# snphbaum/scikit-gpuppy

Hardware: AMD Instinct MI355X
Metric: GP fit+predict pts/sec (K+Cholesky, N=16384 d=8) (higher is better)
Workload: dtype f64; 1 GPU; C3: N=16384 d=8 M=16384 fit(Gram+Cholesky+alpha)+estimate_many, theta fixed; global_batch=32768, parallelism=1 GPU

## Files before the change

scikit-gpuppy_amd/csrc/chol.hip:

```cpp
#include <algorithm>
#include <atomic>
#include <chrono>
#include <cstdio>
#include <cstdlib>
#include <functional>
#include <map>
#include <mutex>
#include <vector>

#include "common.h"

#include "leaf.h"

__attribute__((amdgpu_waves_per_eu(2, 2))) __global__ __launch_bounds__(256) void potrf_trtri128_elim_kernel(double *A, long ld, double *dinv, double *diag_out, int *info,
                                                                 int col_offset, int prio)
{
    __shared__ __attribute__((aligned(16))) double X[36 * XB];
    __shared__ int bad_s;
    if (prio) __builtin_amdgcn_s_setprio(3);
    leaf_elim_body(A, ld, dinv, diag_out, info, col_offset, X, &bad_s);
}

static void leaf_exclusive_setup()
{
    static const bool done = [] {
        (void)hipFuncSetAttribute(reinterpret_cast<const void *>(potrf_trtri128_elim_kernel), hipFuncAttributeMaxDynamicSharedMemorySize, 52 * 1024);
        return true;
    }();
    (void)done;
}

int launch_potrf_leaf(double *A, int64_t ld, double *dinv, double *diag_out, int *info_dev, int col_offset,
                      hipStream_t s, Profiler *prof, int exclusive)
{
    ProfScope ps(prof, s, GPX_K_POTRF_LEAF, (double)TILE * TILE * TILE);
    if (exclusive) leaf_exclusive_setup();
    hipLaunchKernelGGL(potrf_trtri128_elim_kernel, dim3(1), dim3(256), exclusive ? 52 * 1024 : 0, s, A, (long)ld, dinv, diag_out, info_dev, col_offset, 1);
    GPX_HIP(hipGetLastError());
    return 0;
}

extern "C" int gpx_dev_potrf_leaf(double *A, int64_t ld, double *dinv, double *diag_out, int *info_dev, int col_offset,
                                  void *stream)
{
    return launch_potrf_leaf(A, ld, dinv, diag_out, info_dev, col_offset, (hipStream_t)stream, nullptr, 0);
}

static inline int64_t split_point(int64_t nb)
{
    int64_t h = 1;
    while (h * 2 < nb) h *= 2;
    return h;
}

int trsm_right_lt(double *Z, int64_t ldz, int64_t rows, const double *L, int64_t ldl, const double *Dinv,
                  int64_t c0, int64_t c1, hipStream_t s, Profiler *prof)
{
    const int64_t nb = c1 - c0;
    if (nb <= 0 || rows <= 0) return 0;
    if (nb == 1) {
        double *Zc = Z + c0 * TILE;
        return launch_gemm_nt(Zc, ldz, Dinv + c0 * (int64_t)TILE * TILE, TILE, Zc, ldz, rows, TILE, TILE, 1.0, 0.0, 0, s, prof);
    }
    const int64_t h = split_point(nb), cm = c0 + h;
    GPX_TRY(trsm_right_lt(Z, ldz, rows, L, ldl, Dinv, c0, cm, s, prof));
    GPX_TRY(launch_gemm_nt(Z + c0 * TILE, ldz, L + (cm * TILE) * ldl + c0 * TILE, ldl, Z + cm * TILE, ldz, rows,
                           (c1 - cm) * TILE, h * TILE, -1.0, 1.0, 0, s, prof));
    return trsm_right_lt(Z, ldz, rows, L, ldl, Dinv, cm, c1, s, prof);
}

static int trtri_upper_rec(double *Z, int64_t ldz, const double *L, int64_t ldl, const double *Dinv, int64_t c0, int64_t c1,
                           hipStream_t s, Profiler *prof)
{
    const int64_t nb = c1 - c0;
    if (nb <= 0) return 0;
    if (nb == 1) {
        double *Zc = Z + c0 * TILE;
        return launch_gemm_nt(Zc, ldz, Dinv + c0 * (int64_t)TILE * TILE, TILE, Zc, ldz, c1 * TILE, TILE, TILE, 1.0, 0.0, 0, s, prof);
    }
    const int64_t h = split_point(nb), cm = c0 + h;
    GPX_TRY(trtri_upper_rec(Z, ldz, L, ldl, Dinv, c0, cm, s, prof));
    GPX_TRY(launch_gemm_nt(Z + c0 * TILE, ldz, L + (cm * TILE) * ldl + c0 * TILE, ldl, Z + cm * TILE, ldz, cm * TILE,
                           (c1 - cm) * TILE, h * TILE, -1.0, 1.0, 0, s, prof, (int)(c0 * TILE) + 1));
    return trtri_upper_rec(Z, ldz, L, ldl, Dinv, cm, c1, s, prof);
}

int build_linv_t(const double *L, int64_t ld, int64_t nblk, const double *Dinv, double *Z, hipStream_t s, Profiler *prof)
{
    const int64_t npad = nblk * TILE;
    GPX_TRY(launch_set_identity(Z, npad, npad, s));
    return trtri_upper_rec(Z, npad, L, ld, Dinv, 0, nblk, s, prof);
}

int build_kinv_from_factor(const double *L, int64_t ld, int64_t nblk, const double *Dinv, double *Z, double *Kinv,
                           hipStream_t s, Profiler *prof)
{
    const int64_t npad = nblk * TILE;
    GPX_TRY(build_linv_t(L, ld, nblk, Dinv, Z, s, prof));
    GPX_TRY(launch_gemm_nt(Z, npad, Z, npad, Kinv, npad, npad, npad, npad, 1.0, 0.0, 1, s, prof, 1));
    return launch_symmetrize_lower(Kinv, npad, npad, s);
}

static int chol_rec(double *L, int64_t ld, int64_t b0, int64_t b1, double *Dinv, double *diagL, int *info_dev,
                    hipStream_t s, Profiler *prof)
{
    const int64_t nb = b1 - b0;
    if (nb <= 0) return 0;
    if (nb == 1)
        return launch_potrf_leaf(L + (b0 * TILE) * ld + b0 * TILE, ld, Dinv + b0 * (int64_t)TILE * TILE,
                                 diagL + b0 * TILE, info_dev, (int)(b0 * TILE), s, prof, 0);
    const int64_t h = split_point(nb), bm = b0 + h;
    GPX_TRY(chol_rec(L, ld, b0, bm, Dinv, diagL, info_dev, s, prof));
    GPX_TRY(trsm_right_lt(L + (bm * TILE) * ld, ld, (b1 - bm) * TILE, L, ld, Dinv, b0, bm, s, prof));
    const double *A21 = L + (bm * TILE) * ld + b0 * TILE;
    GPX_TRY(launch_gemm_nt(A21, ld, A21, ld, L + (bm * TILE) * ld + bm * TILE, ld, (b1 - bm) * TILE, (b1 - bm) * TILE,
                           h * TILE, -1.0, 1.0, 1, s, prof));
    return chol_rec(L, ld, bm, b1, Dinv, diagL, info_dev, s, prof);
}

constexpr int64_t CHOL_NBP = 8;

int64_t chol_dataflow_state_ints(int64_t nbr);
int64_t chol_dataflow_table_ints(int64_t nbr);
bool chol_dataflow_supported(int64_t nbr);
int64_t chol_dataflow_word_steps();
int64_t chol_dataflow_word_colc(int64_t nbr, int64_t k);
int launch_chol_dataflow(double *L, int64_t ld, int64_t nb, int64_t c0, double *Dinv, double *diag, int *info_dev, int *state_dev,
                         std::vector<int> &host_tab, unsigned long long limit_ticks, hipStream_t s, int workers = 0, int exclusive = 0,
                         const int *tab_ready = nullptr, int first_rows = 0, int extra = 0, const int *gate = nullptr);
int chol_dataflow_fill_tables(int nbr, int first_rows, int *dst, int cap);

static_assert(CHOL_NBP * TILE == CHOL_PANEL_COLS, "common.h: CHOL_PANEL_COLS");

static long env_long(const char *name, long dflt) { const char *e = getenv(name); return e ? atol(e) : dflt; }
static bool debug_enabled() { static const bool v = getenv("GPX_DEBUG") != nullptr; return v; }

static unsigned long long wait_limit_ticks()
{
    static const unsigned long long v = [] { const char *e = getenv("GPX_WAIT_LIMIT_MS"); const double ms = e ? atof(e) : 5000.0; return (unsigned long long)((ms > 0.01 ? ms : 0.01) * 1e5); }();
    return v;
}

__global__ void wait_count_kernel(const int *ctr, int want, unsigned long long limit_ticks, int *stall)
{
    const unsigned long long t0 = __builtin_amdgcn_s_memrealtime();
    while (__hip_atomic_load(ctr, __ATOMIC_RELAXED, __HIP_MEMORY_SCOPE_AGENT) < want) {
        if (__builtin_amdgcn_s_memrealtime() - t0 > limit_ticks) {
            __hip_atomic_store(stall, 1, __ATOMIC_RELAXED, __HIP_MEMORY_SCOPE_AGENT);
            break;
        }
        __builtin_amdgcn_s_sleep(8);
    }
}

static int queue_wait(hipStream_t on, const int *counter, int want, int *stall, unsigned long long limit_ticks = wait_limit_ticks())
{
    hipLaunchKernelGGL(wait_count_kernel, dim3(1), dim3(1), 0, on, counter, want, limit_ticks, stall);
    GPX_HIP(hipGetLastError());
    return 0;
}

struct Events {
    std::vector<hipEvent_t> all;
    Events() = default;
    Events(const Events &) = delete;
    Events &operator=(const Events &) = delete;
    ~Events() { clear(); }
    void clear()
    {
        for (hipEvent_t e : all) (void)hipEventDestroy(e);
        all.clear();
    }
    int make(hipEvent_t *e)
    {
        GPX_HIP(hipEventCreateWithFlags(e, hipEventDisableTiming));
        all.push_back(*e);
        return 0;
    }
};

struct TopPipe {
    hipStream_t stream = nullptr;
    int64_t r0 = 0, r1 = 0;
    Events *events = nullptr;
    const int *colsig = nullptr;
    int colwant = 0;
    int *stall = nullptr;
    const int *sq_state = nullptr;
    int64_t sq_rows = 0;
    int64_t sq_nbr = 0;
    const TopPipe *next = nullptr;
    void follow_square(const int *state, int64_t rows, int64_t below)
    {
        sq_state = state;
        sq_rows = rows;
        sq_nbr = rows + below;
    }
};

static int colsig_wait(const TopPipe *top, int64_t c)
{
    static const bool force_stall = getenv("GPX_TEST_FORCE_STALL") != nullptr;
    static bool forced = false;
    const bool force = force_stall && !forced;
    forced = forced || force;
    return queue_wait(top->stream, top->colsig + c, force ? 0x7fffffff : top->colwant, top->stall, force ? 1000ull : wait_limit_ticks());
}

static int top_column(double *L, int64_t ld, int64_t B0, int64_t j, const double *Dinv, const TopPipe *top, Profiler *prof, int part = 0)
{
    double *Zt = L + (top->r0 * TILE) * ld;
    const int64_t M = (top->r1 - top->r0) * TILE;
    if (top->sq_state && part == 1) return 0;
    if (top->colsig && part != 2) {
        if (!top->sq_state) GPX_TRY(colsig_wait(top, j - B0));
        else if (j == B0)
            for (int64_t c = 0; c < top->sq_rows; ++c) GPX_TRY(colsig_wait(top, c));
    }
    if (top->sq_state) {
        const int64_t B1 = B0 + top->sq_rows;
        GPX_TRY(queue_wait(top->stream, top->sq_state + chol_dataflow_word_steps(), (int)(j - B0 + 1), top->stall));
        GPX_TRY(launch_gemm_nt(Zt + j * TILE, ld, Dinv + j * (int64_t)TILE * TILE, TILE, Zt + j * TILE, ld, M, TILE, TILE, 1.0, 0.0, 0, top->stream, prof));
        if (j + 1 < B1) {
            GPX_TRY(queue_wait(top->stream, top->sq_state + chol_dataflow_word_colc(top->sq_nbr, j - B0), (int)(4 * (B1 - 1 - j)), top->stall));
            GPX_TRY(launch_gemm_nt(Zt + j * TILE, ld, L + ((j + 1) * TILE) * ld + j * TILE, ld, Zt + (j + 1) * TILE, ld, M, (B1 - 1 - j) * TILE, TILE,
                                   -1.0, 1.0, 0, top->stream, prof, 0, 0, 1));
        }
        return 0;
    }
    if (j > B0 && part != 2)
        GPX_TRY(launch_gemm_nt(Zt + B0 * TILE, ld, L + (j * TILE) * ld + B0 * TILE, ld, Zt + j * TILE, ld, M, TILE, (j - B0) * TILE,
                               -1.0, 1.0, 0, top->stream, prof));
    if (part == 1) return 0;
    return launch_gemm_nt(Zt + j * TILE, ld, Dinv + j * (int64_t)TILE * TILE, TILE, Zt + j * TILE, ld, M, TILE, TILE, 1.0, 0.0, 0,
                          top->stream, prof);
}

static int chol_square_steps(double *L, int64_t ld, int64_t B0, int64_t B1, int64_t j0, int64_t j1, double *Dinv,
                             double *diagL, int *info_dev, hipStream_t s, Profiler *prof, const TopPipe *top = nullptr, int excl = 0)
{
    for (int64_t j = j0; j < j1; ++j) {
        for (const TopPipe *t = top; t; t = t->next)
            if (t->stream && t->r1 > t->r0) GPX_TRY(top_column(L, ld, B0, j, Dinv, t, prof, 1));
        GPX_TRY(launch_potrf_leaf(L + (j * TILE) * ld + j * TILE, ld, Dinv + j * (int64_t)TILE * TILE, diagL + j * TILE, info_dev,
                                  (int)(j * TILE), s, prof, excl == 2 || (excl == 1 && j == B0)));
        const int64_t rows_below = B1 - (j + 1);
        if (rows_below > 0) {
            double *Z = L + ((j + 1) * TILE) * ld + j * TILE;
            GPX_TRY(launch_gemm_nt(Z, ld, Dinv + j * (int64_t)TILE * TILE, TILE, Z, ld, rows_below * TILE, TILE, TILE, 1.0, 0.0, 0, s, prof));
            GPX_TRY(launch_gemm_nt(Z, ld, Z, ld, L + ((j + 1) * TILE) * ld + (j + 1) * TILE, ld, rows_below * TILE,
                                   rows_below * TILE, TILE, -1.0, 1.0, 0, s, prof));
        }
        hipEvent_t e = nullptr;
        for (const TopPipe *t = top; t; t = t->next) {
            if (!t->stream || t->r1 <= t->r0) continue;
            if (!e) {
                GPX_TRY(t->events->make(&e));
                GPX_HIP(hipEventRecord(e, s));
            }
            GPX_HIP(hipStreamWaitEvent(t->stream, e, 0));
            GPX_TRY(top_column(L, ld, B0, j, Dinv, t, prof, 2));
        }
    }
    return 0;
}

int chol_panel_factor(double *L, int64_t ld, int64_t nblk_all, int64_t B0, int64_t B1, double *Dinv, double *diagL,
                      int *info_dev, hipStream_t s, Profiler *prof)
{
    GPX_TRY(chol_square_steps(L, ld, B0, B1, B0, B1, Dinv, diagL, info_dev, s, prof));
    if (nblk_all > B1)
        GPX_TRY(trsm_right_lt(L + (B1 * TILE) * ld, ld, (nblk_all - B1) * TILE, L, ld, Dinv, B0, B1, s, prof));
    return 0;
}

static void retire_events(const std::vector<hipEvent_t> &fresh)
{
    static std::mutex mu;
    static std::vector<hipEvent_t> pending;
    std::lock_guard<std::mutex> lk(mu);
    size_t keep = 0;
    for (size_t i = 0; i < pending.size(); ++i) {
        if (hipEventQuery(pending[i]) == hipSuccess) (void)hipEventDestroy(pending[i]);
        else pending[keep++] = pending[i];
    }
    pending.resize(keep);
    pending.insert(pending.end(), fresh.begin(), fresh.end());
}

static void retire_buffers(const std::vector<void *> &bufs, const std::vector<hipStream_t> &behind)
{
    static std::mutex mu;
    struct Pending { std::vector<hipEvent_t> events; std::vector<void *> bufs; };
    static std::vector<Pending> pending;
    std::lock_guard<std::mutex> lk(mu);
    size_t keep = 0;
    for (size_t i = 0; i < pending.size(); ++i) {
        bool done = true;
        for (hipEvent_t e : pending[i].events) done = done && hipEventQuery(e) == hipSuccess;
        if (done) {
            for (hipEvent_t e : pending[i].events) (void)hipEventDestroy(e);
            for (void *q : pending[i].bufs) dfree(q);
        } else {
            if (keep != i) pending[keep] = std::move(pending[i]);
            ++keep;
        }
    }
    pending.resize(keep);
    if (bufs.empty()) return;
    Pending fresh;
    fresh.bufs = bufs;
    for (hipStream_t st : behind) {
        hipEvent_t e = nullptr;
        if (hipEventCreateWithFlags(&e, hipEventDisableTiming) != hipSuccess || hipEventRecord(e, st) != hipSuccess) {
            (void)hipStreamSynchronize(st);
            if (e) (void)hipEventDestroy(e);
            continue;
        }
        fresh.events.push_back(e);
    }
    pending.push_back(std::move(fresh));
}

__global__ void merge_info_kernel(const int *two, int *one)
{
    if (two[1]) atomicMax(one, (int)GPX_INFO_STALLED);
    else if (two[0]) atomicCAS(one, 0, two[0]);
}

static thread_local int g_panel_share = 1;
extern "C" int gpx_dev_set_panel_share(int ranks)
{
    if (ranks < 1) { gpx_set_error("gpx_dev_set_panel_share: ranks must be >= 1"); return GPX_ERR_BAD_ARG; }
    g_panel_share = ranks;
    return 0;
}

static long sqk_from() { static const long v = env_long("GPX_SQK_FROM", -2); return v; }
static bool square_launch_wanted(int64_t b0, int64_t beside, int share, bool from_p)
{
    static const long tiles = env_long("GPX_SQK_TILES", 1000);
    if (sqk_from() == -1 || !chol_dataflow_supported(CHOL_NBP)) return false;
    if (sqk_from() == 0) return true;
    if (sqk_from() > 0 && from_p) return b0 >= sqk_from() * CHOL_NBP;
    return b0 == 0 || beside / share < tiles;
}

int chol_panel_factor_piped(double *L, int64_t ld, int64_t nblk_all, int64_t B0, int64_t B1, double *Dinv, double *diagL,
                            int *info_dev, hipStream_t s, Profiler *prof, const double *P, int64_t ldp, int64_t kp,
                            int64_t hb, hipStream_t sh, hipStream_t sf)
{
    const int64_t c0 = B0 * TILE, w = (B1 - B0) * TILE;
    const bool own_streams = sh && sf;
    double *Csq = L + c0 * ld + c0;
    if (P) GPX_TRY(launch_gemm_nt(P, ldp, P, ldp, Csq, ld, w, w, kp, -1.0, 1.0, 0, s, prof));
    const int64_t nrem = nblk_all - B1;
    const bool sqk = B1 - B0 == CHOL_NBP && B0 % CHOL_NBP == 0 && square_launch_wanted(B0, nrem * (nrem + 1) / 2 + nrem * (B1 - B0), g_panel_share, false);
    std::vector<void *> scratch;
    Events events;
    hipStream_t st_int = nullptr;
    struct Slice { hipStream_t st; int64_t r0, r1; bool joined; };
    std::vector<Slice> slices;
    int *two = nullptr, *state = nullptr, *tab_dev = nullptr;
    auto chain = [&](const TopPipe *top) -> int {
        if (!sqk) return chol_square_steps(L, ld, B0, B1, B0, B1, Dinv, diagL, info_dev, s, prof, top);
        static thread_local std::vector<int> tab;
        GPX_TRY(launch_chol_dataflow(L, ld, B1, B0, Dinv, diagL, two, state, tab, wait_limit_ticks(), s, 32, 1, tab_dev));
        for (int64_t j = B0; j < B1; ++j)
            for (const TopPipe *t = top; t; t = t->next) GPX_TRY(top_column(L, ld, B0, j, Dinv, t, prof));
        return 0;
    };
    auto merge_info = [&](hipStream_t on) -> int {
        if (!sqk) return 0;
        hipLaunchKernelGGL(merge_info_kernel, dim3(1), dim3(1), 0, on, (const int *)two, info_dev);
        GPX_HIP(hipGetLastError());
        return 0;
    };
    auto body = [&]() -> int {
        if (sqk) {
            static thread_local std::vector<int> tab_host;
            const int64_t nstate = chol_dataflow_state_ints(CHOL_NBP), ntab = chol_dataflow_table_ints(CHOL_NBP);
            tab_host.assign((size_t)ntab, 0);
            if (chol_dataflow_fill_tables((int)CHOL_NBP, (int)CHOL_NBP, tab_host.data(), (int)ntab) < 0) { gpx_set_error("chol_panel_factor_piped: task tables"); return GPX_ERR_STATE; }
            double *buf = nullptr;
            GPX_TRY(dalloc(&buf, (4 + nstate + ntab) / 2 + 2));
            scratch.push_back(buf);
            two = reinterpret_cast<int *>(buf); state = two + 4; tab_dev = state + nstate;
            GPX_HIP(hipMemsetAsync(two, 0, sizeof(int) * (size_t)(4 + nstate), s));
            GPX_HIP(hipMemcpyAsync(tab_dev, tab_host.data(), sizeof(int) * (size_t)ntab, hipMemcpyHostToDevice, s));
        }
        if (nrem > 0) {
            if (own_streams) {
                const int64_t h = hb < 0 ? 0 : (hb > nrem ? nrem : hb);
                if (h > 0) slices.push_back({sh, B1, B1 + h, false});
                if (h < nrem) slices.push_back({sf, B1 + h, nblk_all, false});
            } else if ((st_int = stream_acquire(1)) != nullptr) {
                slices.push_back({st_int, B1, nblk_all, true});
            }
        }
        if (slices.empty()) {
            if (nrem > 0 && P) GPX_TRY(launch_gemm_nt(P + w * ldp, ldp, P, ldp, Csq + w * ld, ld, nrem * TILE, w, kp, -1.0, 1.0, 0, s, prof));
            GPX_TRY(chain(nullptr));
            GPX_TRY(merge_info(s));
            return nrem > 0 ? trsm_right_lt(L + (B1 * TILE) * ld, ld, nrem * TILE, L, ld, Dinv, B0, B1, s, prof) : 0;
        }
        std::vector<TopPipe> tops(slices.size());
        hipEvent_t e0 = nullptr;
        GPX_TRY(events.make(&e0));
        GPX_HIP(hipEventRecord(e0, s));
        for (size_t i = 0; i < slices.size(); ++i) {
            const Slice &sl = slices[i];
            GPX_HIP(hipStreamWaitEvent(sl.st, e0, 0));
            if (P) GPX_TRY(launch_gemm_nt(P + (sl.r0 * TILE - c0) * ldp, ldp, P, ldp, L + (sl.r0 * TILE) * ld + c0, ld, (sl.r1 - sl.r0) * TILE, w, kp,
                                          -1.0, 1.0, 0, sl.st, prof));
            TopPipe &top = tops[i];
            top.stream = sl.st; top.r0 = sl.r0; top.r1 = sl.r1; top.events = &events;
            if (sqk) { top.follow_square(state, B1 - B0, 0); top.stall = two + 1; }
            top.next = i + 1 < slices.size() ? &tops[i + 1] : nullptr;
        }
        GPX_TRY(chain(&tops[0]));
        for (const Slice &sl : slices) {
            if (sl.joined) {
                hipEvent_t e1 = nullptr;
                GPX_TRY(events.make(&e1));
                GPX_HIP(hipEventRecord(e1, sl.st));
                GPX_HIP(hipStreamWaitEvent(s, e1, 0));
            } else {
                GPX_TRY(merge_info(sl.st));
            }
        }
        return merge_info(s);
    };
    const int rc = body();
    std::vector<hipStream_t> behind{s};
    for (const Slice &sl : slices) if (!sl.joined) behind.push_back(sl.st);
    if (rc) for (hipStream_t q : behind) (void)hipStreamSynchronize(q);
    if (rc && st_int) (void)hipStreamSynchronize(st_int);
    retire_buffers(scratch, behind);
    retire_events(events.all);
    events.all.clear();
    if (st_int) stream_release(st_int, 1);
    return rc;
}

__global__ __launch_bounds__(256) void cu_blocker_kernel(const int *stop, int *placed, unsigned long long limit_ticks)
{
    asm volatile("v_mov_b32 v255, 0\n\tv_accvgpr_write_b32 a39, 0" ::: "v255", "a39");
    if (threadIdx.x == 0) __hip_atomic_fetch_add(placed, 1, __ATOMIC_RELAXED, __HIP_MEMORY_SCOPE_AGENT);
    if (threadIdx.x < 64) {
        const unsigned long long t0 = __builtin_amdgcn_s_memrealtime();
        while (__hip_atomic_load(stop, __ATOMIC_RELAXED, __HIP_MEMORY_SCOPE_AGENT) == 0 &&
               __builtin_amdgcn_s_memrealtime() - t0 < limit_ticks)
            __builtin_amdgcn_s_sleep(127);
    }
    __syncthreads();
}

__global__ void set_flag_kernel(int *flag, int value) { __hip_atomic_store(flag, value, __ATOMIC_RELAXED, __HIP_MEMORY_SCOPE_AGENT); }

__global__ void wait_placed_kernel(const int *placed, int want, unsigned long long limit_ticks)
{
    const unsigned long long t0 = __builtin_amdgcn_s_memrealtime();
    while (__hip_atomic_load(placed, __ATOMIC_RELAXED, __HIP_MEMORY_SCOPE_AGENT) < want && __builtin_amdgcn_s_memrealtime() - t0 < limit_ticks)
        __builtin_amdgcn_s_sleep(16);
}

namespace {
std::mutex g_conc_mu;
std::map<std::pair<hipStream_t, hipStream_t>, bool> g_conc_seen;
thread_local bool g_force_plain = false;
}
void chol_concurrency_forget()
{
    std::lock_guard<std::mutex> lk(g_conc_mu);
    g_conc_seen.clear();
}
void chol_force_plain_schedule(bool on) { g_force_plain = on; }

static bool streams_run_concurrently(hipStream_t a, hipStream_t b)
{
    if (g_force_plain) return false;
    if (const char *e = getenv("GPX_CONCURRENT_STREAMS")) return atoi(e) != 0;
    if (!a || !b) return false;
    std::lock_guard<std::mutex> lk(g_conc_mu);
    auto it = g_conc_seen.find({a, b});
    if (it != g_conc_seen.end()) return it->second;
    double *wd = nullptr;
    bool good = false;
    if (dalloc(&wd, 2) == 0) {
        int *w = reinterpret_cast<int *>(wd);
        if (hipMemsetAsync(w, 0, 2 * sizeof(int), a) == hipSuccess && hipStreamSynchronize(a) == hipSuccess) {
            hipLaunchKernelGGL(wait_count_kernel, dim3(1), dim3(1), 0, a, (const int *)w, 1, 200000ull, w + 1);
            const bool l1 = hipGetLastError() == hipSuccess;
            hipLaunchKernelGGL(set_flag_kernel, dim3(1), dim3(1), 0, b, w, 1);
            const bool l2 = hipGetLastError() == hipSuccess;
            int h[2] = {0, 1};
            if (hipStreamSynchronize(a) == hipSuccess && hipStreamSynchronize(b) == hipSuccess && l1 && l2 &&
                hipMemcpy(h, w, sizeof(h), hipMemcpyDeviceToHost) == hipSuccess)
                good = (h[1] == 0);
        }
        dfree(wd);
    }
    (void)hipGetLastError();
    if (debug_enabled()) fprintf(stderr, "[gpx] concurrent-streams probe (%p waits, %p releases): %d\n", (void *)a, (void *)b, (int)good);
    g_conc_seen[{a, b}] = good;
    return good;
}
static bool blockers_may_wait_on(hipStream_t s_blk, hipStream_t s, hipStream_t s_pan, hipStream_t s_top)
{
    return streams_run_concurrently(s_blk, s) && streams_run_concurrently(s_blk, s_pan) && (!s_top || streams_run_concurrently(s_blk, s_top));
}

static int reserve_cus() { static const int v = (int)std::min(128L, std::max(0L, env_long("GPX_RESERVE_CUS", 32))); return v; }
static long reserve_below_tiles() { static const long v = env_long("GPX_RESERVE_TILES", 3000); return v; }
static int blocker_stream_prio() { static const int v = (int)env_long("GPX_BLK_PRIO", 1); return v; }
static int sqk_workers() { static const int v = (int)env_long("GPX_SQK_WORKERS", 32); return v; }
static bool trap_enabled() { static const bool v = env_long("GPX_TRAP", 1) != 0; return v; }
static int64_t dflow_max_blocks() { static const int64_t v = env_long("GPX_DFLOW_MAX_BLOCKS", 0); return v; }
static bool dflow_small_enabled() { static const bool v = env_long("GPX_DFLOW_SMALL", 1) != 0; return v; }
constexpr long FIT_EMU_MIN_BLOCKS = 96, FIT_EMU_GROUP = 4;
static int64_t fit_emu_group(int64_t nblk)
{
    static const long on = env_long("GPX_FIT_EMU", -1), group = std::max(1L, env_long("GPX_FIT_EMU_GROUP", FIT_EMU_GROUP));
    if (on == 0 || (on < 0 && nblk < FIT_EMU_MIN_BLOCKS)) return 0;
    const int64_t panels = (nblk + CHOL_NBP - 1) / CHOL_NBP;
    return emu_enabled(CHOL_PANEL_COLS * group) && panels > group ? group : 0;
}

void chol_probe_streams(hipStream_t s, hipStream_t s_pan, hipStream_t s_top)
{
    if (!s_pan) return;
    const bool concurrent = streams_run_concurrently(s_pan, s) && (!s_top || streams_run_concurrently(s_top, s));
    if (!concurrent || reserve_cus() == 0) return;
    hipStream_t s_blk = stream_acquire(blocker_stream_prio());
    if (!s_blk) return;
    (void)blockers_may_wait_on(s_blk, s, s_pan, s_top);
    stream_release(s_blk, blocker_stream_prio());
}

namespace {
struct WholeDataflow {
    std::vector<int> tab;
    Scratch sc;
    double *state = nullptr;
    explicit WholeDataflow(hipStream_t s) : sc(s) {}
    int take(int64_t nblk) { return sc.take(&state, (chol_dataflow_state_ints(nblk) + chol_dataflow_table_ints(nblk)) / 2 + 2); }
    int launch(double *L, int64_t ld, int64_t nblk, double *Dinv, double *diagL, int *info_dev)
    {
        return launch_chol_dataflow(L, ld, nblk, 0, Dinv, diagL, info_dev, reinterpret_cast<int *>(state), tab, wait_limit_ticks(), sc.s, 0, 0);
    }
};

int small_dataflow_factor(double *L, int64_t ld, int64_t nblk, double *Dinv, double *diagL, int *info_dev, hipStream_t s)
{
    WholeDataflow df(s);
    int st_host[2] = {0, 0};
    GPX_TRY(df.take(nblk));
    GPX_HIP(hipMemsetAsync(info_dev + 1, 0, sizeof(int), s));
    GPX_TRY(df.launch(L, ld, nblk, Dinv, diagL, info_dev));
    GPX_HIP(hipMemcpyAsync(st_host, info_dev, 2 * sizeof(int), hipMemcpyDeviceToHost, s));
    GPX_HIP(df.sc.wait_and_free());
    if (!st_host[1]) return 0;
    gpx_set_error("factorisation of a %ld-row block: an in-kernel hand-off timed out (GPX_WAIT_LIMIT_MS); GPX_DFLOW_SMALL=0 selects the launch chain",
                  (long)(nblk * TILE));
    return GPX_ERR_STATE;
}

struct SoloToken {
    int dev = 0; bool solo = false;
    static std::atomic<int> &count(int d) { static std::atomic<int> c[64]; return c[d & 63]; }
    SoloToken() { (void)hipGetDevice(&dev); solo = count(dev).fetch_add(1) == 0; }
    ~SoloToken() { count(dev).fetch_sub(1); }
};

struct Lookahead {
    double *L;
    int64_t ld, nblk;
    double *Dinv, *diagL;
    int *info_dev;
    hipStream_t s, s_pan, s_top;
    Profiler *prof;
    const std::function<int()> *after_fork;
    const std::function<int(int64_t, int64_t, bool)> *panel_final;
    std::vector<int64_t> Bs{0};
    int64_t P = 0;
    SoloToken token;
    bool concurrent = false;
    bool trap_on = false;
    static constexpr int64_t SQK_STATE = 1024, SQK_TAB = 256, SQK_GATE = 1008;
    static constexpr int SQK_EXTRA = 32;
    std::vector<char> sqk_use;
    double *sqk_buf = nullptr;
    std::vector<std::vector<int>> sqk_tabs;
    std::vector<int> sqk_tab_host;
    std::vector<TopPipe> tops;
    int *stall = nullptr, *stop_flag = nullptr, *placed = nullptr, *sig = nullptr;
    hipStream_t s_blk = nullptr;
    int nres = 0;
    bool reserved = false, released = false;
    bool blk_gone = false;
    int64_t G = 0;
    EmuFrame esy;
    bool sq_split_prev = false;
    Events events;
    hipEvent_t ev0 = nullptr, ev_blk = nullptr, ev_blk_gone = nullptr;
    std::vector<hipEvent_t> ev_pf, ev_next, ev_top, ev_tu, ev_first, ev_sqp;
    double host_t0 = 0.0;
    std::vector<double> host_marks;
    static double host_now() { return std::chrono::duration<double, std::micro>(std::chrono::steady_clock::now().time_since_epoch()).count(); }
    void mark() { if (debug_enabled()) host_marks.push_back(host_now() - host_t0); }
    ~Lookahead()
    {
        if (debug_enabled()) {
            fprintf(stderr, "[gpx] host enqueue marks, panel by panel (us): ");
            for (double m : host_marks) fprintf(stderr, "%.0f ", m);
            fprintf(stderr, "\n");
        }
        release_blockers();
        if (s_top) (void)hipStreamSynchronize(s_top);
        (void)hipStreamSynchronize(s_pan);
        if (s_blk) {
            (void)hipStreamSynchronize(s);
            (void)hipStreamSynchronize(s_blk);
            stream_release(s_blk, blocker_stream_prio());
        }
        (void)hipStreamSynchronize(s);
        events.clear();
        if (sqk_buf) dfree(sqk_buf);
        emu_free(esy);
    }
    int64_t bnd(int64_t p) const { return Bs[std::min<int64_t>(p, P)]; }
    int64_t far_blk(int64_t p) const { return G ? bnd((p / G + 1) * G) : nblk; }
    bool boundary(int64_t p) const { return G && (p + 1) % G == 0 && p + 1 < P; }
    int64_t bulk_tiles(int64_t p) const
    {
        const int64_t nrem = nblk - bnd(p + 2), wt = std::max<int64_t>(0, std::min(nrem, far_blk(p) - bnd(p + 2)));
        return nrem <= 0 ? 0 : wt * (wt + 1) / 2 + (nrem - wt) * wt;
    }
    int64_t beside_tiles(int64_t pp) const
    {
        if (pp == 0 || boundary(pp - 1)) return 0;
        return (nblk - bnd(pp + 1)) * (bnd(pp + 1) - bnd(pp)) + bulk_tiles(pp - 1);
    }
    int hook(int64_t p, int64_t slack, bool last) const { return panel_final ? (*panel_final)(p, slack, last) : 0; }
    bool piped(int64_t q) const { return s_top && bnd(q + 1) < nblk; }
    bool use_sqk(int64_t pp) const { return pp >= 0 && pp < P && sqk_use[(size_t)pp]; }
    int *sqk_state(int64_t pp) const { return reinterpret_cast<int *>(sqk_buf) + pp * SQK_STATE; }
    int *sqk_tab(int64_t pp) const { return reinterpret_cast<int *>(sqk_buf) + P * SQK_STATE + pp * SQK_TAB; }
    int *sqk_gate(int64_t pp) const { return sqk_state(pp) + SQK_GATE; }
    int64_t sqk_below(int64_t pp) const { return s_top ? bnd(pp + 2) - bnd(pp + 1) : 0; }
    bool top_late(int64_t p) const { return piped(p) && use_sqk(p) && sqk_below(p) == bnd(p + 2) - bnd(p + 1) && bnd(p + 2) > bnd(p + 1); }
    bool q_on_chain(int64_t p) const { return sq_split_prev && piped(p); }
    int setup()
    {
        while (Bs.back() < nblk) Bs.push_back(std::min<int64_t>(nblk, Bs.back() + CHOL_NBP));
        P = (int64_t)Bs.size() - 1;
        stall = info_dev + 1;
        stop_flag = info_dev + 2;
        placed = info_dev + 3;
        sig = info_dev + 4;
        concurrent = token.solo && streams_run_concurrently(s_pan, s) && (!s_top || streams_run_concurrently(s_top, s));
        trap_on = trap_enabled() && concurrent;
        G = fit_emu_group(nblk);
        if (G) {
            esy.reserve(emu_syrk_plan((nblk - bnd(G)) * TILE, (int64_t)CHOL_PANEL_COLS * G));
            if (emu_alloc(esy, nullptr)) G = 0;
        }
        sqk_use.assign((size_t)P, 0);
        for (int64_t pp = 0; concurrent && pp < P; ++pp)
            sqk_use[(size_t)pp] = square_launch_wanted(bnd(pp), beside_tiles(pp), 1, true);
        sqk_tabs.resize((size_t)P);
        tops.resize((size_t)P + 1);
        if (std::count(sqk_use.begin(), sqk_use.end(), 1)) GPX_TRY(dalloc(&sqk_buf, (P * SQK_STATE + P * SQK_TAB) / 2 + 2));
        for (std::vector<hipEvent_t> *v : {&ev_pf, &ev_next, &ev_top, &ev_tu, &ev_first, &ev_sqp}) v->resize((size_t)P + 1);
        GPX_TRY(events.make(&ev0));
        for (int64_t p = 0; p < P; ++p)
            for (hipEvent_t *e : {&ev_pf[p], &ev_next[p], &ev_top[p], &ev_tu[p], &ev_first[p], &ev_sqp[p]}) GPX_TRY(events.make(e));
        GPX_TRY(events.make(&ev_top[P]));
        nres = concurrent ? reserve_cus() : 0;
        s_blk = nres ? stream_acquire(blocker_stream_prio()) : nullptr;
        if (s_blk && !blockers_may_wait_on(s_blk, s, s_pan, s_top)) {
            stream_release(s_blk, blocker_stream_prio());
            s_blk = nullptr;
        }
        if (s_blk) GPX_TRY(events.make(&ev_blk));
        if (s_blk && G) GPX_TRY(events.make(&ev_blk_gone));
        host_t0 = debug_enabled() ? host_now() : 0.0;
        return 0;
    }
    int sqk_launch(int64_t pp, int64_t Ba, int64_t Bb)
    {
        const int64_t below = sqk_below(pp);
        return launch_chol_dataflow(L, ld, Bb + below, Ba, Dinv, diagL, info_dev, sqk_state(pp), sqk_tabs[(size_t)pp], wait_limit_ticks(), s_pan,
                                    std::min<int>(sqk_workers(), (int)(4 * (Bb - Ba - 1) + 4)), 1, sqk_tab(pp), (int)(Bb - Ba),
                                    below > 0 ? SQK_EXTRA : 0, sqk_gate(pp));
    }
    void sqk_open_gate(int64_t pp, hipStream_t on)
    {
        if (use_sqk(pp) && sqk_below(pp) > 0) hipLaunchKernelGGL(set_flag_kernel, dim3(1), dim3(1), 0, on, sqk_gate(pp), 1);
    }
    void follow_square(int64_t q) { tops[(size_t)q].follow_square(sqk_state(q), bnd(q + 1) - bnd(q), sqk_below(q)); }
    void release_blockers()
    {
        if (!reserved || released) return;
        hipLaunchKernelGGL(set_flag_kernel, dim3(1), dim3(1), 0, s, stop_flag, 1);
        released = true;
    }
    int drop_reservation()
    {
        if (!reserved) return 0;
        release_blockers();
        GPX_HIP(hipEventRecord(ev_blk_gone, s_blk));
        reserved = released = false;
        blk_gone = true;
        return 0;
    }
    int reserve_now(int64_t p)
    {
        const int64_t nrem = nblk - bnd(p + 2);
        if (!s_blk || reserved || nrem <= 0 || bulk_tiles(p) >= reserve_below_tiles() || (sqk_from() < 0 && use_sqk(p + 1))) return 0;
        if (blk_gone) GPX_HIP(hipStreamWaitEvent(s, ev_blk_gone, 0));
        blk_gone = false;
        GPX_HIP(hipMemsetAsync(stop_flag, 0, 2 * sizeof(int), s));
        GPX_HIP(hipEventRecord(ev_blk, s));
        GPX_HIP(hipStreamWaitEvent(s_blk, ev_blk, 0));
        const double expect_s = (double)(nblk * TILE) * (double)(nblk * TILE) * (double)(nblk * TILE) / 3.0 / 20e12;
        const unsigned long long limit = (unsigned long long)((0.05 + 4.0 * expect_s) * 1e8);
        hipLaunchKernelGGL(cu_blocker_kernel, dim3((unsigned)nres), dim3(256), 0, s_blk, (const int *)stop_flag, placed, limit);
        hipLaunchKernelGGL(wait_placed_kernel, dim3(1), dim3(1), 0, s, (const int *)placed, nres, 20000ull);
        GPX_HIP(hipGetLastError());
        reserved = true;
        return 0;
    }
    int prepare()
    {
        if (trap_on) GPX_HIP(hipMemsetAsync(sig, 0, sizeof(int) * (size_t)(P * CHOL_NBP), s));
        if (sqk_buf) {
            sqk_tab_host.assign((size_t)(P * SQK_TAB), 0);
            for (int64_t pp = 0; pp < P; ++pp) {
                const int rows = (int)(bnd(pp + 1) - bnd(pp)), nbr = rows + (int)sqk_below(pp);
                if (use_sqk(pp) && (chol_dataflow_state_ints(nbr) > SQK_GATE || chol_dataflow_fill_tables(nbr, rows, sqk_tab_host.data() + pp * SQK_TAB, (int)SQK_TAB) < 0)) {
                    gpx_set_error("chol_factor: square launch of %d + %d block rows does not fit its state / table slot", rows, nbr - rows);
                    return GPX_ERR_STATE;
                }
            }
            GPX_HIP(hipMemsetAsync(sqk_buf, 0, sizeof(int) * (size_t)(P * SQK_STATE), s));
            GPX_HIP(hipMemcpyAsync(sqk_tab(0), sqk_tab_host.data(), sizeof(int) * sqk_tab_host.size(), hipMemcpyHostToDevice, s));
        }
        sqk_open_gate(0, s);
        GPX_HIP(hipEventRecord(ev0, s));
        GPX_HIP(hipStreamWaitEvent(s_pan, ev0, 0));
        for (int64_t q = 0; q < P; ++q) {
            tops[q].stream = piped(q) ? s_top : nullptr;
            tops[q].r0 = bnd(q + 1) + (use_sqk(q) ? sqk_below(q) : 0);
            tops[q].r1 = nblk;
            tops[q].events = &events;
        }
        if (piped(0)) GPX_HIP(hipStreamWaitEvent(s_top, ev0, 0));
        return 0;
    }
    int first_panel()
    {
        if (use_sqk(0)) {
            GPX_TRY(sqk_launch(0, 0, bnd(1)));
            follow_square(0);
            if (after_fork) GPX_TRY((*after_fork)());
            if (tops[0].stream && tops[0].r1 > tops[0].r0)
                for (int64_t j = 0; j < bnd(1); ++j) GPX_TRY(top_column(L, ld, 0, j, Dinv, &tops[0], prof));
        } else {
            GPX_TRY(chol_square_steps(L, ld, 0, bnd(1), 0, 1, Dinv, diagL, info_dev, s_pan, prof, &tops[0], 0));
            if (after_fork) GPX_TRY((*after_fork)());
            GPX_TRY(chol_square_steps(L, ld, 0, bnd(1), 1, bnd(1), Dinv, diagL, info_dev, s_pan, prof, &tops[0], 2));
        }
        if (piped(0)) GPX_HIP(hipEventRecord(ev_top[0], s_top));
        GPX_HIP(hipEventRecord(ev_pf[0], s_pan));
        return 0;
    }
    int square_update(int64_t p)
    {
        const int64_t B0 = bnd(p), B1 = bnd(p + 1), B2 = bnd(p + 2);
        const bool late = top_late(p), on_chain = q_on_chain(p);
        if (piped(p) && !late) GPX_HIP(hipStreamWaitEvent(s, ev_top[p], 0));
        else if (!piped(p)) GPX_TRY(trsm_right_lt(L + (B1 * TILE) * ld, ld, (nblk - B1) * TILE, L, ld, Dinv, B0, B1, s, prof));
        const double *Ptop = L + (B1 * TILE) * ld + B0 * TILE;
        if (on_chain) {
            GPX_HIP(hipStreamWaitEvent(s_pan, ev_sqp[p - 1], 0));
            if (!late) GPX_HIP(hipStreamWaitEvent(s_pan, ev_top[p], 0));
        }
        GPX_TRY(launch_gemm_nt(Ptop, ld, Ptop, ld, L + (B1 * TILE) * ld + B1 * TILE, ld, (B2 - B1) * TILE, (B2 - B1) * TILE, (B1 - B0) * TILE,
                               -1.0, 1.0, 1, on_chain ? s_pan : s, prof));
        if (!on_chain) GPX_HIP(hipEventRecord(ev_next[p], s));
        if (sqk_from() < 0 && use_sqk(p + 1)) release_blockers();
        return 0;
    }
    int start_chain(int64_t q)
    {
        const int64_t p = q - 1, B1 = bnd(q), B2 = bnd(q + 1);
        if (!q_on_chain(p)) GPX_HIP(hipStreamWaitEvent(s_pan, ev_next[p], 0));
        if (use_sqk(q)) return sqk_launch(q, B1, B2);
        GPX_TRY(chol_square_steps(L, ld, B1, B2, B1, B1 + 1, Dinv, diagL, info_dev, s_pan, prof, nullptr, (reserved || B2 >= nblk) ? 1 : 0));
        if (piped(q)) GPX_HIP(hipEventRecord(ev_first[p], s_pan));
        return 0;
    }
    int trailing_update(int64_t p)
    {
        const int64_t B0 = bnd(p), B1 = bnd(p + 1), B2 = bnd(p + 2), B3 = bnd(p + 3), K = (B1 - B0) * TILE, nrem = nblk - B2;
        if (top_late(p)) GPX_HIP(hipStreamWaitEvent(s, ev_top[p], 0));
        sq_split_prev = false;
        if (nrem <= 0) return 0;
        const double *Ptop = L + (B1 * TILE) * ld + B0 * TILE;
        const double *Pr = L + (B2 * TILE) * ld + B0 * TILE;
        int merged = GPX_ERR_STATE;
        constexpr long trap_min = 1024;
        const int64_t fc = std::min(nblk, std::max(B2, far_blk(p))), wt = fc - B2;
        if (trap_on && bulk_tiles(p) >= trap_min && B2 - B1 == CHOL_NBP)
            merged = launch_syrk_trap_signal(Pr, ld, Ptop, ld, L + (B2 * TILE) * ld + B1 * TILE, ld, nrem * TILE, (B2 - B1) * TILE, K, -1.0, 1.0,
                                             sig + p * CHOL_NBP, s, prof, wt * TILE);
        if (merged != 0 && merged != GPX_ERR_STATE) return merged;
        if (merged != 0)
            GPX_TRY(launch_gemm_nt(Pr, ld, Ptop, ld, L + (B2 * TILE) * ld + B1 * TILE, ld, nrem * TILE, (B2 - B1) * TILE,
                                   K, -1.0, 1.0, 0, s, prof, 0, 0, (use_sqk(p + 1) && p + 1 > 0) ? 1 : 0));
        sqk_open_gate(p + 1, s);
        if (piped(p + 1)) {
            TopPipe &top = tops[(size_t)p + 1];
            if (merged == 0) {
                top.colsig = sig + p * CHOL_NBP;
                top.colwant = (int)nrem;
                top.stall = stall;
            } else {
                GPX_HIP(hipEventRecord(ev_tu[p], s));
                GPX_HIP(hipStreamWaitEvent(s_top, ev_tu[p], 0));
            }
            if (use_sqk(p + 1)) follow_square(p + 1);
            else GPX_HIP(hipStreamWaitEvent(s_top, ev_first[p], 0));
            GPX_TRY(top_column(L, ld, B1, B1, Dinv, &top, prof));
        }
        if (merged != 0 && wt < nrem) {
            if (wt > 0) {
                GPX_TRY(launch_gemm_nt(Pr, ld, Pr, ld, L + (B2 * TILE) * ld + B2 * TILE, ld, (B3 - B2) * TILE, (B3 - B2) * TILE, K, -1.0, 1.0, 1, s, prof));
                GPX_HIP(hipEventRecord(ev_sqp[p], s));
                sq_split_prev = true;
                if (B3 < fc)
                    GPX_TRY(launch_gemm_nt(Pr + ((B3 - B2) * TILE) * ld, ld, Pr, ld, L + (B3 * TILE) * ld + B2 * TILE, ld, (fc - B3) * TILE, wt * TILE, K,
                                           -1.0, 1.0, 1, s, prof));
                GPX_TRY(launch_gemm_nt(Pr + (wt * TILE) * ld, ld, Pr, ld, L + (fc * TILE) * ld + B2 * TILE, ld, (nblk - fc) * TILE, wt * TILE, K, -1.0, 1.0, 0,
                                       s, prof));
            }
        } else if (merged != 0 && p + 2 < P && B3 > B2) {
            GPX_TRY(launch_gemm_nt(Pr, ld, Pr, ld, L + (B2 * TILE) * ld + B2 * TILE, ld, (B3 - B2) * TILE, (B3 - B2) * TILE, K, -1.0, 1.0, 1, s, prof));
            GPX_HIP(hipEventRecord(ev_sqp[p], s));
            sq_split_prev = true;
            if (B3 < nblk)
                GPX_TRY(launch_gemm_nt(Pr + ((B3 - B2) * TILE) * ld, ld, Pr, ld, L + (B3 * TILE) * ld + B2 * TILE, ld, (nblk - B3) * TILE,
                                       nrem * TILE, K, -1.0, 1.0, 1, s, prof));
        } else if (merged != 0)
            GPX_TRY(launch_gemm_nt(Pr, ld, Pr, ld, L + (B2 * TILE) * ld + B2 * TILE, ld, nrem * TILE, nrem * TILE, K, -1.0, 1.0, 1, s, prof));
        if (B3 >= nblk) release_blockers();
        return 0;
    }
    int group_boundary(int64_t p)
    {
        const int64_t g0 = bnd(p + 1 - G), B1 = bnd(p + 1), rows = (nblk - B1) * TILE, K = (B1 - g0) * TILE;
        if (piped(p)) GPX_HIP(hipStreamWaitEvent(s, ev_top[p], 0));
        else GPX_TRY(trsm_right_lt(L + (B1 * TILE) * ld, ld, (nblk - B1) * TILE, L, ld, Dinv, bnd(p), B1, s, prof));
        GPX_TRY(drop_reservation());
        sq_split_prev = false;
        double *C = L + (B1 * TILE) * ld + B1 * TILE;
        esy.use(emu_syrk_plan(rows, K));
        GPX_TRY(emu_syrk_split(esy, L + (B1 * TILE) * ld + g0 * TILE, ld, rows, s));
        GPX_TRY(emu_syrk_panel(esy, 0, C, ld, rows, s, prof, TILE));
        GPX_HIP(hipEventRecord(ev_next[p], s));
        GPX_TRY(start_chain(p + 1));
        sqk_open_gate(p + 1, s);
        if (piped(p + 1)) {
            GPX_HIP(hipEventRecord(ev_tu[p], s));
            GPX_HIP(hipStreamWaitEvent(s_top, ev_tu[p], 0));
            if (use_sqk(p + 1)) follow_square(p + 1);
            else GPX_HIP(hipStreamWaitEvent(s_top, ev_first[p], 0));
            GPX_TRY(top_column(L, ld, B1, B1, Dinv, &tops[(size_t)p + 1], prof));
        }
        for (int64_t q = 1; q * CHOL_PANEL_COLS < rows; ++q) GPX_TRY(emu_syrk_panel(esy, q, C, ld, rows, s, prof, TILE));
        return 0;
    }
    int finish_chain(int64_t q)
    {
        const int64_t B1 = bnd(q), B2 = bnd(q + 1);
        const TopPipe &top = tops[(size_t)q];
        if (!use_sqk(q))
            GPX_TRY(chol_square_steps(L, ld, B1, B2, B1 + 1, B2, Dinv, diagL, info_dev, s_pan, prof, &top, (reserved || bnd(q + 2) >= nblk) ? 2 : 0));
        else if (top.stream && top.r1 > top.r0)
            for (int64_t j = B1 + 1; j < B2; ++j) GPX_TRY(top_column(L, ld, B1, j, Dinv, &top, prof));
        if (piped(q)) GPX_HIP(hipEventRecord(ev_top[q], s_top));
        GPX_HIP(hipEventRecord(ev_pf[q], s_pan));
        return 0;
    }
};
}

int chol_factor(double *L, int64_t ld, int64_t nblk, double *Dinv, double *diagL, int *info_dev, hipStream_t s,
                hipStream_t s_pan, Profiler *prof, hipStream_t s_top, const std::function<int()> *after_fork,
                const std::function<int(int64_t, int64_t, bool)> *panel_final)
{
    const int64_t last = (nblk + CHOL_NBP - 1) / CHOL_NBP - 1;
    const bool lookahead = nblk > CHOL_NBP && s_pan != nullptr;
    const bool whole = !g_force_plain && chol_dataflow_supported(nblk);
    if (!lookahead) {
        if (after_fork) GPX_TRY((*after_fork)());
        if (whole && nblk > CHOL_NBP && nblk <= 64 && dflow_small_enabled())
            GPX_TRY(small_dataflow_factor(L, ld, nblk, Dinv, diagL, info_dev, s));
        else
            GPX_TRY((nblk <= CHOL_NBP) ? chol_panel_factor(L, ld, nblk, 0, nblk, Dinv, diagL, info_dev, s, prof)
                                       : chol_rec(L, ld, 0, nblk, Dinv, diagL, info_dev, s, prof));
        if (panel_final) GPX_TRY((*panel_final)(last, 0, true));
        return 0;
    }
    if (whole && nblk <= dflow_max_blocks()) {
        SoloToken token;
        WholeDataflow df(s);
        GPX_TRY(df.take(nblk));
        if (after_fork) GPX_TRY((*after_fork)());
        GPX_TRY(df.launch(L, ld, nblk, Dinv, diagL, info_dev));
        if (panel_final) GPX_TRY((*panel_final)(last, 0, true));
        return 0;
    }
    Lookahead la{L, ld, nblk, Dinv, diagL, info_dev, s, s_pan, s_top, prof, after_fork, panel_final};
    GPX_TRY(la.setup());
    GPX_TRY(la.prepare());
    GPX_TRY(la.first_panel());
    for (int64_t p = 0; p <= last; ++p) {
        GPX_HIP(hipStreamWaitEvent(s, la.ev_pf[p], 0));
        if (p == last) return la.hook(p, 0, true);
        if (la.boundary(p)) GPX_TRY(la.group_boundary(p));
        else {
            GPX_TRY(la.reserve_now(p));
            GPX_TRY(la.square_update(p));
            GPX_TRY(la.start_chain(p + 1));
            GPX_TRY(la.trailing_update(p));
        }
        GPX_TRY(la.hook(p, (nblk - la.bnd(p + 2) + CHOL_NBP - 1) / CHOL_NBP, false));
        GPX_TRY(la.finish_chain(p + 1));
        la.mark();
    }
    return 0;
}
```

Baseline: 496,200 pts/s.

## Defer and interleave emulated SYRK panel launches across lookahead panels

At a group boundary, only the first emulated SYRK panels are enqueued. The remaining far-trailing panels are deferred and spread over the following panel iterations: the near panels (up to G) are flushed before each trailing update, and the far ones are paced in proportion to progress. The aim is to keep the critical panel chain and square updates from queuing behind a large batch of far SYRK work on the main stream. It is enabled only for concurrent, grouped runs with at most 192 blocks, and it makes the enqueue order more intricate, which raises the risk of dependency-ordering mistakes.

Result: no change. 497,900 pts/s (median of 4 runs) (+0.3%).

```diff
diff --git a/scikit-gpuppy_amd/csrc/chol.hip b/scikit-gpuppy_amd/csrc/chol.hip
--- a/scikit-gpuppy_amd/csrc/chol.hip
+++ b/scikit-gpuppy_amd/csrc/chol.hip
@@ -525,6 +525,13 @@
     if (on == 0 || (on < 0 && nblk < FIT_EMU_MIN_BLOCKS)) return 0;
     const int64_t panels = (nblk + CHOL_NBP - 1) / CHOL_NBP;
     return emu_enabled(CHOL_PANEL_COLS * group) && panels > group ? group : 0;
+}
+constexpr int64_t FIT_EMU_ORDER_MAX_BLOCKS = 192;
+static int fit_emu_order(int64_t nblk)
+{
+    static const long v = env_long("GPX_FIT_EMU_ORDER", -1);
+    if (v >= 0) return (int)std::min(2L, v);
+    return nblk <= FIT_EMU_ORDER_MAX_BLOCKS ? 2 : 0;
 }
 
 void chol_probe_streams(hipStream_t s, hipStream_t s_pan, hipStream_t s_top)
@@ -601,6 +608,9 @@
     bool blk_gone = false;
     int64_t G = 0;
     EmuFrame esy;
+    int order = 0;
+    int64_t pend_q = 0, pend_n = 0, pend_rows = 0, pend_p = 0;
+    double *pend_C = nullptr;
     bool sq_split_prev = false;
     Events events;
     hipEvent_t ev0 = nullptr, ev_blk = nullptr, ev_blk_gone = nullptr;
@@ -666,6 +676,7 @@
             esy.reserve(emu_syrk_plan((nblk - bnd(G)) * TILE, (int64_t)CHOL_PANEL_COLS * G));
             if (emu_alloc(esy, nullptr)) G = 0;
         }
+        order = concurrent && G >= 2 ? fit_emu_order(nblk) : 0;
         sqk_use.assign((size_t)P, 0);
         for (int64_t pp = 0; concurrent && pp < P; ++pp)
             sqk_use[(size_t)pp] = square_launch_wanted(bnd(pp), beside_tiles(pp), 1, true);
@@ -861,6 +872,7 @@
     int group_boundary(int64_t p)
     {
         const int64_t g0 = bnd(p + 1 - G), B1 = bnd(p + 1), rows = (nblk - B1) * TILE, K = (B1 - g0) * TILE;
+        GPX_TRY(queue_pending(pend_n));
         if (piped(p)) GPX_HIP(hipStreamWaitEvent(s, ev_top[p], 0));
         else GPX_TRY(trsm_right_lt(L + (B1 * TILE) * ld, ld, (nblk - B1) * TILE, L, ld, Dinv, bnd(p), B1, s, prof));
         GPX_TRY(drop_reservation());
@@ -879,7 +891,29 @@
             else GPX_HIP(hipStreamWaitEvent(s_top, ev_first[p], 0));
             GPX_TRY(top_column(L, ld, B1, B1, Dinv, &tops[(size_t)p + 1], prof));
         }
-        for (int64_t q = 1; q * CHOL_PANEL_COLS < rows; ++q) GPX_TRY(emu_syrk_panel(esy, q, C, ld, rows, s, prof, TILE));
+        pend_C = C;
+        pend_p = p;
+        pend_rows = rows;
+        pend_q = 1;
+        pend_n = (rows + CHOL_PANEL_COLS - 1) / CHOL_PANEL_COLS;
+        return queue_pending(order ? 2 : pend_n);
+    }
+    int queue_pending(int64_t upto)
+    {
+        for (upto = std::min(upto, pend_n); pend_q < upto; ++pend_q) GPX_TRY(emu_syrk_panel(esy, pend_q, pend_C, ld, pend_rows, s, prof, TILE));
+        return 0;
+    }
+    double far_rows(int64_t q) const { return (double)(pend_rows - q * CHOL_PANEL_COLS); }
+    int far_behind(int64_t p)
+    {
+        if (order < 2 || pend_q >= pend_n || !(use_sqk(p + 1) || (reserved && !released))) return 0;
+        double total = 0.0, done = 0.0;
+        for (int64_t q = G; q < pend_n; ++q) (q < pend_q ? done : total) += far_rows(q);
+        const double target = (total + done) * (double)(p - pend_p) / (double)(G - 1);
+        while (pend_q < pend_n && done < target) {
+            done += far_rows(pend_q);
+            GPX_TRY(queue_pending(pend_q + 1));
+        }
         return 0;
     }
     int finish_chain(int64_t q)
@@ -929,13 +963,18 @@
     GPX_TRY(la.first_panel());
     for (int64_t p = 0; p <= last; ++p) {
         GPX_HIP(hipStreamWaitEvent(s, la.ev_pf[p], 0));
-        if (p == last) return la.hook(p, 0, true);
+        if (p == last) {
+            GPX_TRY(la.queue_pending(la.pend_n));
+            return la.hook(p, 0, true);
+        }
         if (la.boundary(p)) GPX_TRY(la.group_boundary(p));
         else {
             GPX_TRY(la.reserve_now(p));
             GPX_TRY(la.square_update(p));
             GPX_TRY(la.start_chain(p + 1));
+            GPX_TRY(la.queue_pending(la.order == 1 ? la.pend_n : la.G));
             GPX_TRY(la.trailing_update(p));
+            GPX_TRY(la.far_behind(p));
         }
         GPX_TRY(la.hook(p, (nblk - la.bnd(p + 2) + CHOL_NBP - 1) / CHOL_NBP, false));
         GPX_TRY(la.finish_chain(p + 1));
```
